# zhu-xlab/tomosar2height

Measured on AMD Instinct MI355X. Metric: training tiles/sec (Berlin crop, cloud-only), higher is better.
Workload: dtype f32; 1 GPU; BASELINE.json configs[1]: Berlin cloud-only, fp32 per-point GEMMs, train_step(tile) per tile, 4 tiles coalesced per forward/backward (Trainer default), N=131072 points/tile, R=256, ALTO depth 5, 512x512 target, optimize_every=64; points_per_tile=131072, optimize_every=64, train_batch=1, coalesce_tiles=4, optimizer=t2h FlatAdamW (one kernel over the flat bucket), parallelism=dp1, rccl_ranks=0, channels_last=True, point_distribution=70 % in 160 buildings + 30 % uniform, grid_convs=conv_bx3.hip: fp32 products from 3 fp16 MFMAs (2-way split, block scales), library_fallbacks=0, hip_graph=False

## Files before the change

### tomosar2height_amd/csrc/conv_bx3.hip

```cpp
#include <stdlib.h>
#include "t2h_common.h"
#include "gemm_args.h"
#include "gemm_tile.h"

namespace t2h {
namespace {

using bf16x8 = __attribute__((ext_vector_type(8))) __bf16;
using f16x8 = __attribute__((ext_vector_type(8))) _Float16;
using f16x2 = __attribute__((ext_vector_type(2))) _Float16;
using bf16x2 = __attribute__((ext_vector_type(2))) __bf16;
using f32x2 = __attribute__((ext_vector_type(2))) float;
using s16x4 = __attribute__((ext_vector_type(4))) short;
using s16x8 = __attribute__((ext_vector_type(8))) short;
typedef __attribute__((address_space(3))) void lds_void;
typedef const __attribute__((address_space(1))) void glb_void;
typedef __attribute__((address_space(3))) s16x4 lds_s16x4;

#ifndef T2H_BX3_BDIRECT
#define T2H_BX3_BDIRECT 1
#endif
constexpr int NT = 256;
constexpr int TW = 32;
constexpr int CC = 32;
// ... 491 lines not shown
        if (t + 1 < T) prefetch(t + 1, pre_m[(t + 1) & 1], pre_o[(t + 1) & 1]);
#pragma unroll
        for (int z = 0; z < 16; ++z)
            patch[((z & 3) + 8 * (z >> 2) + 4 * h) * 36 + r] = H2 ? ldexpf(acc[i][j][z] * winv, -e_cur) : acc[i][j][z];
        float4 bv = make_float4(0.f, 0.f, 0.f, 0.f);
        {
            int col, co;
            tile_off(t, 0, col, co);
            if (p.bias) bv = *reinterpret_cast<const float4 *>(p.bias + co);
        }
#pragma unroll
        for (int pass = 0; pass < 4; ++pass) {
            float4 v = *reinterpret_cast<const float4 *>(patch + (pass * 8 + er) * 36 + ec);
            int col, co;
            const size_t q = tile_off(t, pass, col, co);
            const float4 mk = pre_m[t & 1][pass];
            float4 old = pre_o[t & 1][pass];
            if (rank1 && p.mask) {
                old.x = mk.x > 0.f ? old.x : 0.f; old.y = mk.y > 0.f ? old.y : 0.f;
                old.z = mk.z > 0.f ? old.z : 0.f; old.w = mk.w > 0.f ? old.w : 0.f;
            }
            v.x += bv.x; v.y += bv.y; v.z += bv.z; v.w += bv.w;
            if (UPM == 1) {
                float4 *dst = reinterpret_cast<float4 *>(p.y + q);
                if (accum) { v.x += old.x; v.y += old.y; v.z += old.z; v.w += old.w; }
                if (p.addend) { v.x += mk.x; v.y += mk.y; v.z += mk.z; v.w += mk.w; }
                *dst = v;
                continue;
            }
            if (p.mask) {
                v.x = mk.x > 0.f ? v.x : 0.f; v.y = mk.y > 0.f ? v.y : 0.f;
                v.z = mk.z > 0.f ? v.z : 0.f; v.w = mk.w > 0.f ? v.w : 0.f;
            }
            if (relu) { v.x = relu1(v.x); v.y = relu1(v.y); v.z = relu1(v.z); v.w = relu1(v.w); }
            float4 *dst = reinterpret_cast<float4 *>(ybase + q * p.ldy + col);
            if (accum) { v.x += old.x; v.y += old.y; v.z += old.z; v.w += old.w; }
            *dst = v;
        }
    }
  }
}

struct WgradArgs {
    const float *dy;
    const float *x;
    float *slab;
    float *colslab;
    int H, W, Cin, Cout;
    int n_units, units_per_split;
    int ldx;
    int lddy;
};

template <int COT, int NPL, bool UP = false, int GT = 0>
__global__ __launch_bounds__(NT, 2) void bx3_wgrad_kernel(WgradArgs p) {
    static_assert(!(UP && GT), "UP and GT are different forms");
    constexpr int NTAPS = GT ? GT : (UP ? 4 : 9);
    constexpr int WPC = 4 / COT;
    constexpr int TMAX = (NTAPS + WPC - 1) / WPC;
    constexpr int YS = COT == 1 ? 64 : 64 * COT + 64;
    constexpr int XS = 64;
    constexpr int YPLANE = 32 * YS, XHP = GT ? GT * TW : (UP ? 4 * TW : 3 * (TW + 2)), XPLANE = XHP * XS;
    constexpr int LDS_WORK = NPL * YPLANE + NPL * XPLANE;
    constexpr int LDS_BYTES = LDS_WORK >= 4 * 32 * 36 * 4 ? LDS_WORK : 4 * 32 * 36 * 4;
    constexpr bool H2 = NPL == 2;
    __shared__ __attribute__((aligned(1024))) unsigned char lds[LDS_BYTES + (H2 ? 64 : 0)];
    unsigned char *yimg = lds, *ximg = lds + NPL * YPLANE;
    float *slots = reinterpret_cast<float *>(lds + LDS_BYTES);

    const int tid = threadIdx.x, lane = tid & 63, wave = tid >> 6;
    const int split = GT ? blockIdx.z : blockIdx.x, ci0 = GT ? 0 : blockIdx.y * CC, co0 = (GT ? blockIdx.x : blockIdx.z) * (32 * COT);
    const int u_beg = split * p.units_per_split, u_end = min(p.n_units, u_beg + p.units_per_split);
    const int segs = p.W / TW;

    const int cot = wave / WPC, sub = wave % WPC;
    const int tap_lo = (NTAPS * sub + WPC - 1) / WPC, tap_hi = (NTAPS * (sub + 1) + WPC - 1) / WPC;

    constexpr int XF4 = XHP * 8, XPER = (XF4 + NT - 1) / NT;
    constexpr int YPER = COT;
    float4 xr[XPER], yr[YPER];
    auto load_unit = [&](int u) {
        const int xs = u % segs, row = u / segs;
        const int y = row & (p.H - 1), x0 = xs * TW;
#pragma unroll
        for (int f = 0; f < XPER; ++f) {
            const int idx = tid + f * NT;
            const int px = idx >> 3, c4 = idx & 7;
            const int hy = px / (TW + 2), hx = px - hy * (TW + 2);
            const int gy = y + hy - 1, gx = x0 + hx - 1;
            float4 v = make_float4(0.f, 0.f, 0.f, 0.f);
            if (GT) {
                if (idx < XF4) v = *reinterpret_cast<const float4 *>(p.x + ((size_t)u * TW + (px % TW)) * p.ldx + (px / TW) * 32 + c4 * 4);
            } else if (UP) {
                v = *reinterpret_cast<const float4 *>(p.x + ((size_t)(2 * row + (px >> 6)) * (2 * p.W) + 2 * x0 + (px & 63)) * p.ldx + ci0 + c4 * 4);
            } else if (idx < XF4 && (unsigned)gy < (unsigned)p.H && (unsigned)gx < (unsigned)p.W)
                v = *reinterpret_cast<const float4 *>(p.x + ((size_t)(row + hy - 1) * p.W + gx) * p.ldx + ci0 + c4 * 4);
            xr[f] = v;
        }
#pragma unroll
        for (int f = 0; f < YPER; ++f) {
            const int idx = tid + f * NT;
            const int px = idx / (8 * COT), c4 = idx % (8 * COT);
            yr[f] = *reinterpret_cast<const float4 *>(p.dy + ((size_t)row * p.W + x0 + px) * (GT ? p.lddy : p.Cout) + co0 + c4 * 4);
        }
    };
    float4 csum = make_float4(0.f, 0.f, 0.f, 0.f);
    const bool do_colsum = p.colslab != nullptr && (UP ? blockIdx.z == 0 : blockIdx.y == 0);
    int s_run = E_UNSET, ex_cur = 0, ey_cur = 0;
    auto publish_unit_max = [&](int parity) {
        float mx = 0.f, my = 0.f;
#pragma unroll
        for (int f = 0; f < XPER; ++f) mx = abs4max(mx, xr[f]);
#pragma unroll
        for (int f = 0; f < YPER; ++f) my = abs4max(my, yr[f]);
        mx = wave_max(mx);
        my = wave_max(my);
        if (lane == 0) { slots[(parity * 4 + wave) * 2] = mx; slots[(parity * 4 + wave) * 2 + 1] = my; }
    };
    auto store_unit = [&]() {
#pragma unroll
        for (int f = 0; f < XPER; ++f) {
            const int idx = tid + f * NT;
            if (idx < XF4) {
                const int c4 = idx & 7;
                int px = idx >> 3;
                if (UP) {
                    px = ((px >> 6) * 2 + (px & 1)) * TW + ((px & 63) >> 1);
                    if (do_colsum) { csum.x += xr[f].x; csum.y += xr[f].y; csum.z += xr[f].z; csum.w += xr[f].w; }
                }
                unsigned a1, a2, a3, b1, b2, b3;
                unsigned char *d = ximg + px * XS + c4 * 8;
                if (H2) {
                    split2h(xr[f].x, xr[f].y, ex_cur, a1, a2);
                    split2h(xr[f].z, xr[f].w, ex_cur, b1, b2);
                    *reinterpret_cast<uint2 *>(d) = make_uint2(a1, b1);
                    *reinterpret_cast<uint2 *>(d + XPLANE) = make_uint2(a2, b2);
                    continue;
                }
                split3(xr[f].x, xr[f].y, a1, a2, a3);
                split3(xr[f].z, xr[f].w, b1, b2, b3);
                *reinterpret_cast<uint2 *>(d) = make_uint2(a1, b1);
                if (NPL == 3) {
                    *reinterpret_cast<uint2 *>(d + XPLANE) = make_uint2(a2, b2);
                    *reinterpret_cast<uint2 *>(d + 2 * XPLANE) = make_uint2(a3, b3);
                }
            }
        }
#pragma unroll
        for (int f = 0; f < YPER; ++f) {
            const int idx = tid + f * NT;
            const int px = idx / (8 * COT), c4 = idx % (8 * COT);
            unsigned a1, a2, a3, b1, b2, b3;
            unsigned char *d = yimg + px * YS + c4 * 8;
            if (!UP && do_colsum) { csum.x += yr[f].x; csum.y += yr[f].y; csum.z += yr[f].z; csum.w += yr[f].w; }
            if (H2) {
                split2h(yr[f].x, yr[f].y, ey_cur, a1, a2);
                split2h(yr[f].z, yr[f].w, ey_cur, b1, b2);
                *reinterpret_cast<uint2 *>(d) = make_uint2(a1, b1);
                *reinterpret_cast<uint2 *>(d + YPLANE) = make_uint2(a2, b2);
                continue;
            }
            split3(yr[f].x, yr[f].y, a1, a2, a3);
            split3(yr[f].z, yr[f].w, b1, b2, b3);
            *reinterpret_cast<uint2 *>(d) = make_uint2(a1, b1);
            if (NPL == 3) {
                *reinterpret_cast<uint2 *>(d + YPLANE) = make_uint2(a2, b2);
                *reinterpret_cast<uint2 *>(d + 2 * YPLANE) = make_uint2(a3, b3);
            }
        }
    };

    f32x16 acc[TMAX];
#pragma unroll
    for (int t = 0; t < TMAX; ++t)
#pragma unroll
        for (int z = 0; z < 16; ++z) acc[t][z] = 0.0f;

    const int g = lane >> 4, gi = lane & 15, gq = gi >> 2, gp = gi & 3;
    const int kpix = 8 * (g >> 1) + gq;
    const int choff = (16 * (g & 1) + 4 * gp) * 2;
    auto tr8 = [&](const unsigned char *a, int row_stride) -> bf16x8 {
        const s16x4 lo = __builtin_amdgcn_ds_read_tr16_b64_v4i16((lds_s16x4 *)(a));
        const s16x4 hi = __builtin_amdgcn_ds_read_tr16_b64_v4i16((lds_s16x4 *)(a + 4 * row_stride));
        const s16x8 v = __builtin_shufflevector(lo, hi, 0, 1, 2, 3, 4, 5, 6, 7);
        return *reinterpret_cast<const bf16x8 *>(&v);
    };

    if (u_beg < u_end) load_unit(u_beg);
    if (H2) {
        if (u_beg < u_end) publish_unit_max(u_beg & 1);
        __syncthreads();
    }
    for (int u = u_beg; u < u_end; ++u) {
        if (H2) {
            const float *sl = slots + (u & 1) * 8;
            const int ex_nat = block_exponent(__float_as_uint(fmaxf(fmaxf(sl[0], sl[2]), fmaxf(sl[4], sl[6]))));
            const int ey_nat = block_exponent(__float_as_uint(fmaxf(fmaxf(sl[1], sl[3]), fmaxf(sl[5], sl[7]))));
            if (ex_nat != E_UNSET && ey_nat != E_UNSET && ex_nat + ey_nat < s_run) {
                if (s_run != E_UNSET) {
#pragma unroll
                    for (int t = 0; t < TMAX; ++t)
#pragma unroll
                        for (int z = 0; z < 16; ++z) acc[t][z] = ldexpf(acc[t][z], ex_nat + ey_nat - s_run);
                }
                s_run = ex_nat + ey_nat;
            }
            ex_cur = ex_nat == E_UNSET ? 0 : ex_nat;
            ey_cur = ey_nat == E_UNSET ? 0 : (s_run == E_UNSET ? ey_nat : min(s_run - ex_cur, ey_nat));
        }
        store_unit();
        if (u + 1 < u_end) load_unit(u + 1);
        __syncthreads();
#pragma unroll
        for (int s = 0; s < 2; ++s) {
            bf16x8 af[NPL];
            const unsigned char *ya = yimg + (16 * s + kpix) * YS + cot * 64 + choff;
#pragma unroll
            for (int pl = 0; pl < NPL; ++pl) af[pl] = tr8(ya + pl * YPLANE, YS);
#pragma unroll
            for (int t = 0; t < TMAX; ++t) {
                const int tap = tap_lo + t;
                if (tap < tap_hi) {
                    const int ky = tap / 3, kx = tap - 3 * ky;
                    const unsigned char *xa = ximg + ((UP || GT) ? tap * TW + 16 * s + kpix : ky * (TW + 2) + 16 * s + kpix + kx) * XS + choff;
                    bf16x8 bfr[NPL];
#pragma unroll
                    for (int pl = 0; pl < NPL; ++pl) bfr[pl] = tr8(xa + pl * XPLANE, XS);
                    constexpr int ia[6] = {2, 0, 1, 1, 0, 0}, ib[6] = {0, 2, 1, 0, 1, 0};
                    if (H2) {
#pragma unroll
                        for (int e = 3; e < 6; ++e)
                            acc[t] = __builtin_amdgcn_mfma_f32_32x32x16_f16(*reinterpret_cast<const f16x8 *>(&af[ia[e]]),
                                                                            *reinterpret_cast<const f16x8 *>(&bfr[ib[e]]), acc[t], 0, 0, 0);
                    } else {
#pragma unroll
                        for (int e = (NPL == 3 ? 0 : 5); e < 6; ++e)
                            acc[t] = __builtin_amdgcn_mfma_f32_32x32x16_bf16(af[ia[e]], bfr[ib[e]], acc[t], 0, 0, 0);
                    }
                }
            }
        }
        if (H2 && u + 1 < u_end) publish_unit_max((u + 1) & 1);
        __syncthreads();
    }

    if (do_colsum) {
        float4 *red = reinterpret_cast<float4 *>(lds);
        red[tid] = csum;
        __syncthreads();
        constexpr int CG = UP ? 8 : 8 * COT;
        if (tid < CG) {
            float4 tsum = red[tid];
            for (int j = tid + CG; j < NT; j += CG) { tsum.x += red[j].x; tsum.y += red[j].y; tsum.z += red[j].z; tsum.w += red[j].w; }
            if (UP) *reinterpret_cast<float4 *>(p.colslab + (size_t)split * p.Cin + ci0 + tid * 4) = tsum;
            else *reinterpret_cast<float4 *>(p.colslab + (size_t)split * p.Cout + co0 + tid * 4) = tsum;
        }
        __syncthreads();
    }

    float *patch = reinterpret_cast<float *>(lds) + wave * (32 * 36);
    const int er = lane >> 3, ec = (lane & 7) * 4, r = lane & 31, h = lane >> 5;
    float *sbase = p.slab + (size_t)split * p.Cout * NTAPS * p.Cin;
#pragma unroll
    for (int t = 0; t < TMAX; ++t) {
        const int tap = tap_lo + t;
        if (tap < tap_hi) {
#pragma unroll
            for (int z = 0; z < 16; ++z)
                patch[((z & 3) + 8 * (z >> 2) + 4 * h) * 36 + r] = H2 ? ldexpf(acc[t][z], s_run == E_UNSET ? 0 : -s_run) : acc[t][z];
#pragma unroll
            for (int pass = 0; pass < 4; ++pass) {
                const float4 v = *reinterpret_cast<const float4 *>(patch + (pass * 8 + er) * 36 + ec);
                const int co = co0 + cot * 32 + pass * 8 + er;
                *reinterpret_cast<float4 *>(sbase + ((size_t)co * NTAPS + tap) * p.Cin + ci0 + ec) = v;
            }
        }
    }
}

bool al16(const void *q) { return (uintptr_t)q % 16 == 0; }
bool pow2(int v) { return v > 0 && (v & (v - 1)) == 0; }

int check_bx3(const char *what, int B, int H, int W, int Cin, int Cout) {
    if (B < 1 || !pow2(H) || !pow2(W) || H < 4 || W < TW || H > 32768 || W > 32768 || Cin < 32 || Cout < 32 || Cin % 32 || Cout % 32)
        return fail(T2H_ERR_ARG, "%s: needs power-of-two H >= 4, W >= 32 and Cin, Cout multiples of 32 (B=%d H=%d W=%d %d->%d)", what, B,
                    H, W, Cin, Cout);
    if ((long long)B * H * W > (1LL << 30)) return fail(T2H_ERR_ARG, "%s: more than 2^30 pixels", what);
    return T2H_OK;
}

struct RowsPlan { bool tall; int bn, splits, chunks_per_split; long long tiles; };
RowsPlan bx3_rows_plan(int B, int H, int W, int Kc, int Nc, int ntap = 9, int upm = 0) {
    RowsPlan r{};
    r.bn = Nc % 128 == 0 ? 128 : (Nc % 64 == 0 ? 64 : 32);
    if (upm) {
        r.tall = false;
        const long long row_tiles = (long long)B * (H / 4) * (W / TW);
        if (upm == 1) while (r.bn > 32 && row_tiles * (Nc / r.bn) < 192) r.bn >>= 1;
        r.tiles = row_tiles * (Nc / r.bn);
        r.splits = 1;
        const int nchunk_u = Kc / 64;
        static const long long target_u = 512;
        if (upm == 2 && r.tiles < target_u / 2) {
            long long want = (target_u + r.tiles - 1) / r.tiles;
            if (want > nchunk_u) want = nchunk_u;
            if (want > 32) want = 32;
            r.splits = (int)(want < 1 ? 1 : want);
        }
        r.chunks_per_split = (nchunk_u + r.splits - 1) / r.splits;
        r.splits = (nchunk_u + r.chunks_per_split - 1) / r.chunks_per_split;
        return r;
    }
    static const long long min_tiles8 = env_ll("T2H_BX3_TILES8", 1024);
    const long long tiles8 = H % 8 == 0 ? (long long)B * (H / 8) * (W / TW) * (Nc / r.bn) : 0;
    r.tall = tiles8 >= min_tiles8 && !(ntap == 1 && r.bn == 128);
    r.tiles = r.tall ? tiles8 : (long long)B * (H / 4) * (W / TW) * (Nc / r.bn);
    static const bool narrow = env_flag("T2H_BX3_NARROW", true);
    if (narrow && !r.tall && r.bn == 128 && r.tiles < 256 && Kc <= 128) { r.bn = 64; r.tiles *= 2; }
    r.splits = 1;
    const int nchunk = ntap == 9 ? Kc / (r.tall ? 16 : 32) : Kc / (r.tall ? 32 : 64);
    static const long long target = env_ll("T2H_BX3_ROWS_WGS", 512);
    if (!r.tall && r.tiles < target / 2) {
        long long want = (target + r.tiles - 1) / r.tiles;
        if (want > nchunk) want = nchunk;
        if (want > 32) want = 32;
// ... 50 lines not shown
        e.accum = a.flags & F_ACCUM; e.relu_out = a.flags & F_RELU_OUT;
        a.y = static_cast<float *>(ws); a.bias = nullptr; a.mask = nullptr; a.flags = 0; a.ldy = a.Nc;
    }
    a.splits = r.splits; a.chunks_per_split = r.chunks_per_split; a.ntn_per_wg = 1;
    if (upm == 1) {
        if (r.bn == 128) BX3_LAUNCH_UP(128, 2, 2, 1);
        else if (r.bn == 64) BX3_LAUNCH_UP(64, 4, 1, 1);
        else BX3_LAUNCH_UP(32, 4, 1, 1);
    } else if (upm == 2) {
        if (r.bn == 128) BX3_LAUNCH_UP(128, 2, 2, 2);
        else if (r.bn == 64) BX3_LAUNCH_UP(64, 4, 1, 2);
        else BX3_LAUNCH_UP(32, 4, 1, 2);
    } else if (ntap == 9) {
        if (r.tall) {
            if (r.bn == 128) BX3_LAUNCH(8, 128, 2, 2, 16, 9);
            else if (r.bn == 64) BX3_LAUNCH(8, 64, 4, 1, 16, 9);
            else BX3_LAUNCH(8, 32, 4, 1, 16, 9);
        } else {
            if (r.bn == 128) BX3_LAUNCH(4, 128, 2, 2, 32, 9);
            else if (r.bn == 64) BX3_LAUNCH(4, 64, 4, 1, 32, 9);
            else BX3_LAUNCH(4, 32, 4, 1, 32, 9);
        }
    } else if (ntap == 1 && upm == 0 && npl == 2 && a.Kc == 64 && r.splits == 1 && a.Nc / r.bn >= 8 && persist_n_enabled()) {
        const long long row_tiles = (long long)a.B * (a.H / 4) * (a.W / TW);
        const int pbn = r.bn == 128 ? 64 : r.bn;
        const int ntn = a.Nc / pbn;
        static const long long persist_wgs = env_ll("T2H_BX3_PERSIST_WGS", 2048);
        static const long long min_groups = env_ll("T2H_BX3_PERSIST_MIN_GROUPS", 4);
        long long groups = persist_wgs / (row_tiles > 0 ? row_tiles : 1);
        if (groups < min_groups) groups = min_groups;
        if (groups < 1) groups = 1;
        if (groups > ntn) groups = ntn;
        a.ntn_per_wg = (int)((ntn + groups - 1) / groups);
        groups = (ntn + a.ntn_per_wg - 1) / a.ntn_per_wg;
        const long long pgrid = row_tiles * groups;
        if (pbn == 64) { hipLaunchKernelGGL((bx3_rows_kernel<4, 64, 4, 1, 64, 2, 1, 0, true>), dim3((unsigned)pgrid), dim3(NT), 0, s, a); note_kernel("bx3_rows_kernel<4,64,4,1,64,2,1,0,true>"); }
        else { hipLaunchKernelGGL((bx3_rows_kernel<4, 32, 4, 1, 64, 2, 1, 0, true>), dim3((unsigned)pgrid), dim3(NT), 0, s, a); note_kernel("bx3_rows_kernel<4,32,4,1,64,2,1,0,true>"); }
    } else {
        if (r.tall) {
            if (r.bn == 128) BX3_LAUNCH(8, 128, 2, 2, 32, 1);
            else if (r.bn == 64) BX3_LAUNCH(8, 64, 4, 1, 32, 1);
            else BX3_LAUNCH(8, 32, 4, 1, 32, 1);
        } else {
            if (r.bn == 128) BX3_LAUNCH(4, 128, 2, 2, 64, 1);
            else if (r.bn == 64) BX3_LAUNCH(4, 64, 4, 1, 64, 1);
            else BX3_LAUNCH(4, 32, 4, 1, 64, 1);
        }
    }
    if (int rc = check_launch(what)) return rc;
    if (r.splits > 1) return launch_reduce_rows_epilogue(static_cast<const float *>(ws), r.splits, M * a.Nc, M, a.Nc, e, s);
    return T2H_OK;
}

struct WgradPlan { int cot, splits, units_per_split, n_units; };
WgradPlan bx3_wgrad_plan(int B, int H, int W, int Cin, int Cout) {
    WgradPlan p{};
    p.cot = Cout % 128 == 0 ? 4 : (Cout % 64 == 0 ? 2 : 1);
    p.n_units = B * H * (W / TW);
    const long long groups = (long long)(Cin / CC) * (Cout / (32 * p.cot));
    static const long long forced = env_ll("T2H_BX3_WGRAD_WGS", 0);
    const long long target = forced > 0 ? forced : ((long long)H * W <= 128 * 128 ? 256 : 512);
    long long splits = target / groups;
    if (splits < 1) splits = 1;
    if (splits > p.n_units) splits = p.n_units;
    p.units_per_split = (int)((p.n_units + splits - 1) / splits);
    p.splits = (p.n_units + p.units_per_split - 1) / p.units_per_split;
    return p;
}

}
}

using namespace t2h;

T2H_API int t2h_conv3x3_bx3_supported(int B, int H, int W, int Cin, int Cout) {
    return B >= 1 && pow2(H) && pow2(W) && H >= 4 && W >= TW && H <= 32768 && W <= 32768 && Cin >= 32 && Cout >= 32 && Cin % 32 == 0 &&
           Cout % 32 == 0 && (long long)B * H * W <= (1LL << 30);
}

T2H_API size_t t2h_conv3x3_bx3_weights_bytes(int Cin, int Cout) {
    if (Cin < 32 || Cout < 32 || Cin % 32 || Cout % 32) return 0;
    return (size_t)Cout * 9 * Cin * 6;
}

T2H_API int t2h_conv3x3_bx3_prepare(const float *w, int Cin, int Cout, int transposed, void *wf, t2h_stream_t stream) {
    if (!w || !wf) return fail(T2H_ERR_ARG, "conv3x3_bx3_prepare: null pointer");
    if (Cin < 32 || Cout < 32 || Cin % 32 || Cout % 32 || !al16(wf))
        return fail(T2H_ERR_ARG, "conv3x3_bx3_prepare: Cin=%d, Cout=%d must be multiples of 32, wf 16-byte aligned", Cin, Cout);
    const int Kc = transposed ? Cout : Cin, Nc = transposed ? Cin : Cout;
    const long long total = (long long)(Kc / 16) * 9 * (Nc / 32) * 64;
    const unsigned blocks = (unsigned)((total + 255) / 256);
    if (transposed) hipLaunchKernelGGL(bx3_prepare_kernel<true>, dim3(blocks), dim3(256), 0, as_stream(stream), w, Cin, Cout, static_cast<unsigned *>(wf));
    else hipLaunchKernelGGL(bx3_prepare_kernel<false>, dim3(blocks), dim3(256), 0, as_stream(stream), w, Cin, Cout, static_cast<unsigned *>(wf));
    return check_launch("conv3x3_bx3_prepare");
}

T2H_API size_t t2h_conv3x3_bx3_fwd_workspace_bytes(int B, int H, int W, int Cin, int Cout) {
    if (!t2h_conv3x3_bx3_supported(B, H, W, Cin, Cout)) return 0;
    const RowsPlan r = bx3_rows_plan(B, H, W, Cin, Cout);
    return r.splits > 1 ? (size_t)r.splits * B * H * W * Cout * sizeof(float) : 0;
}

T2H_API size_t t2h_conv3x3_bx3_dgrad_workspace_bytes(int B, int H, int W, int Cin, int Cout) {
    if (!t2h_conv3x3_bx3_supported(B, H, W, Cin, Cout)) return 0;
    const RowsPlan r = bx3_rows_plan(B, H, W, Cout, Cin);
    return r.splits > 1 ? (size_t)r.splits * B * H * W * Cin * sizeof(float) : 0;
}

T2H_API int t2h_conv3x3_bx3_fwd(const float *x, const void *wf, const float *bias, float *y, int B, int H, int W, int Cin, int Cout,
                                int flags, void *workspace, size_t workspace_bytes, t2h_stream_t stream) {
    if (!x || !wf || !y) return fail(T2H_ERR_ARG, "conv3x3_bx3_fwd: null pointer");
    if (int rc = check_bx3("conv3x3_bx3_fwd", B, H, W, Cin, Cout)) return rc;
// ... 11 lines not shown
    if (!dy || !wf_t || !dx) return fail(T2H_ERR_ARG, "conv3x3_bx3_dgrad: null pointer");
    if (int rc = check_bx3("conv3x3_bx3_dgrad", B, H, W, Cin, Cout)) return rc;
    if (!al16(dy) || !al16(wf_t) || !al16(dx) || (mask && !al16(mask))) return fail(T2H_ERR_ARG, "conv3x3_bx3_dgrad: pointers must be 16-byte aligned");
    RowsArgs a{};
    a.x = dy; a.wf = static_cast<const unsigned *>(wf_t); a.bias = nullptr; a.mask = mask; a.y = dx;
    a.B = B; a.H = H; a.W = W; a.Kc = Cout; a.Nc = Cin; a.ldx = Cout; a.ldy = Cin; a.ldm = Cin;
    a.flags = (flags & T2H_ACCUM) ? F_ACCUM : 0;
    a.wscale = f16_trailer(wf_t, (size_t)Cout * 9 * Cin * 4);
    return launch_rows(a, npl_of(flags), workspace, workspace_bytes, as_stream(stream), "conv3x3_bx3_dgrad");
}

T2H_API int t2h_conv3x3_bx3_dgrad_rank1_supported(int B, int H, int W, int Cin, int Cout) {
    if (!t2h_conv3x3_bx3_supported(B, H, W, Cin, Cout)) return 0;
    return bx3_rows_plan(B, H, W, Cout, Cin).splits == 1;
}

T2H_API int t2h_conv3x3_bx3_dgrad_rank1(const float *dy, const void *wf_t, float *dx, const float *mask, const float *g, const float *w1,
                                        int B, int H, int W, int Cin, int Cout, int flags, t2h_stream_t stream) {
    if (!dy || !wf_t || !dx || !g || !w1) return fail(T2H_ERR_ARG, "conv3x3_bx3_dgrad_rank1: null pointer");
    if (int rc = check_bx3("conv3x3_bx3_dgrad_rank1", B, H, W, Cin, Cout)) return rc;
    if (!t2h_conv3x3_bx3_dgrad_rank1_supported(B, H, W, Cin, Cout))
        return fail(T2H_ERR_ARG, "conv3x3_bx3_dgrad_rank1: this shape splits its reduction (use t2h_conv3x3_bx3_dgrad with T2H_ACCUM)");
    if (flags & T2H_ACCUM) return fail(T2H_ERR_ARG, "conv3x3_bx3_dgrad_rank1: the rank-1 term takes the place of the accumulated values");
    if (!al16(dy) || !al16(wf_t) || !al16(dx) || (mask && !al16(mask)) || !al16(w1))
        return fail(T2H_ERR_ARG, "conv3x3_bx3_dgrad_rank1: pointers must be 16-byte aligned");
    RowsArgs a{};
    a.x = dy; a.wf = static_cast<const unsigned *>(wf_t); a.bias = nullptr; a.mask = mask; a.y = dx;
    a.B = B; a.H = H; a.W = W; a.Kc = Cout; a.Nc = Cin; a.ldx = Cout; a.ldy = Cin; a.ldm = Cin;
    a.flags = 0; a.r1_g = g; a.r1_w = w1;
    a.wscale = f16_trailer(wf_t, (size_t)Cout * 9 * Cin * 4);
    return launch_rows(a, npl_of(flags), nullptr, 0, as_stream(stream), "conv3x3_bx3_dgrad_rank1");
}

T2H_API size_t t2h_conv3x3_bx3_wgrad_workspace_bytes(int B, int H, int W, int Cin, int Cout) {
    if (!t2h_conv3x3_bx3_supported(B, H, W, Cin, Cout)) return 0;
    WgradPlan p = bx3_wgrad_plan(B, H, W, Cin, Cout);
    return (size_t)p.splits * ((size_t)Cout * 9 * Cin + Cout) * sizeof(float);
}

T2H_API int t2h_conv3x3_bx3_wgrad(const float *dy, const float *x, float *dw, float *db, int B, int H, int W, int Cin, int Cout,
                                  int flags, void *workspace, size_t workspace_bytes, t2h_stream_t stream) {
    if (!dy || !x || !dw) return fail(T2H_ERR_ARG, "conv3x3_bx3_wgrad: null pointer");
    if (int rc = check_bx3("conv3x3_bx3_wgrad", B, H, W, Cin, Cout)) return rc;
    if (!al16(dy) || !al16(x)) return fail(T2H_ERR_ARG, "conv3x3_bx3_wgrad: pointers must be 16-byte aligned");
    const size_t need = t2h_conv3x3_bx3_wgrad_workspace_bytes(B, H, W, Cin, Cout);
    if (!workspace || workspace_bytes < need || !al16(workspace))
        return fail(T2H_ERR_WORKSPACE, "conv3x3_bx3_wgrad: workspace %zu < %zu bytes", workspace_bytes, need);
    hipStream_t s = as_stream(stream);
    WgradPlan p = bx3_wgrad_plan(B, H, W, Cin, Cout);
    const int Ncols = 9 * Cin;
    float *slab = static_cast<float *>(workspace);
    float *colslab = slab + (size_t)p.splits * Cout * Ncols;
    WgradArgs a{};
    a.dy = dy; a.x = x; a.slab = slab; a.colslab = db ? colslab : nullptr;
    a.H = H; a.W = W; a.Cin = Cin; a.Cout = Cout; a.n_units = p.n_units; a.units_per_split = p.units_per_split; a.ldx = Cin;
    dim3 grid(p.splits, Cin / CC, Cout / (32 * p.cot));
    if (grid.y > 65535 || grid.z > 65535) return fail(T2H_ERR_ARG, "conv3x3_bx3_wgrad: too many channel chunks");
    if (flags & T2H_F16X2) {
        if (p.cot == 4) { hipLaunchKernelGGL((bx3_wgrad_kernel<4, 2>), grid, dim3(NT), 0, s, a); note_kernel("bx3_wgrad_kernel<4,2,false,0>"); }
        else if (p.cot == 2) { hipLaunchKernelGGL((bx3_wgrad_kernel<2, 2>), grid, dim3(NT), 0, s, a); note_kernel("bx3_wgrad_kernel<2,2,false,0>"); }
        else { hipLaunchKernelGGL((bx3_wgrad_kernel<1, 2>), grid, dim3(NT), 0, s, a); note_kernel("bx3_wgrad_kernel<1,2,false,0>"); }
    } else if (flags & T2H_BF16) {
        if (p.cot == 4) { hipLaunchKernelGGL((bx3_wgrad_kernel<4, 1>), grid, dim3(NT), 0, s, a); note_kernel("bx3_wgrad_kernel<4,1,false,0>"); }
        else if (p.cot == 2) { hipLaunchKernelGGL((bx3_wgrad_kernel<2, 1>), grid, dim3(NT), 0, s, a); note_kernel("bx3_wgrad_kernel<2,1,false,0>"); }
        else { hipLaunchKernelGGL((bx3_wgrad_kernel<1, 1>), grid, dim3(NT), 0, s, a); note_kernel("bx3_wgrad_kernel<1,1,false,0>"); }
    } else {
        if (p.cot == 4) { hipLaunchKernelGGL((bx3_wgrad_kernel<4, 3>), grid, dim3(NT), 0, s, a); note_kernel("bx3_wgrad_kernel<4,3,false,0>"); }
        else if (p.cot == 2) { hipLaunchKernelGGL((bx3_wgrad_kernel<2, 3>), grid, dim3(NT), 0, s, a); note_kernel("bx3_wgrad_kernel<2,3,false,0>"); }
        else { hipLaunchKernelGGL((bx3_wgrad_kernel<1, 3>), grid, dim3(NT), 0, s, a); note_kernel("bx3_wgrad_kernel<1,3,false,0>"); }
    }
    if (int rc = check_launch("conv3x3_bx3_wgrad")) return rc;
    return launch_reduce_slabs(slab, p.splits, (long long)Cout * Ncols, Cout, Ncols, Ncols, (flags & T2H_ACCUM) ? 1 : 0, dw, colslab, db, s,
                               0, 0, (flags & T2H_DEFER_REDUCE) != 0);
}

T2H_API int t2h_gemm_bx3_supported(int64_t M, int K, int N) {
    return M >= 128 && M % 128 == 0 && M <= (1LL << 30) && K >= 64 && K % 64 == 0 && N >= 32 && N % 32 == 0;
}

T2H_API size_t t2h_gemm_bx3_weights_bytes(int K, int N) {
    if (K < 16 || N < 32 || K % 16 || N % 32) return 0;
    return (size_t)K * N * 6;
}

T2H_API int t2h_gemm_bx3_prepare(const float *w, int ldw, int K, int N, int w_is_kn, void *wf, t2h_stream_t stream) {
    if (!w || !wf) return fail(T2H_ERR_ARG, "gemm_bx3_prepare: null pointer");
    if (K < 16 || N < 32 || K % 16 || N % 32 || !al16(wf) || ldw < (w_is_kn ? N : K))
        return fail(T2H_ERR_ARG, "gemm_bx3_prepare: K=%d must be a multiple of 16, N=%d of 32, ldw=%d at least the row length", K, N, ldw);
    const long long total = (long long)(K / 16) * (N / 32) * 64;
    const unsigned blocks = (unsigned)((total + 255) / 256);
    if (w_is_kn) hipLaunchKernelGGL(bx3_prepare_gemm_kernel<true>, dim3(blocks), dim3(256), 0, as_stream(stream), w, K, N, ldw, static_cast<unsigned *>(wf));
    else hipLaunchKernelGGL(bx3_prepare_gemm_kernel<false>, dim3(blocks), dim3(256), 0, as_stream(stream), w, K, N, ldw, static_cast<unsigned *>(wf));
    return check_launch("gemm_bx3_prepare");
}

T2H_API size_t t2h_gemm_bx3_workspace_bytes(int64_t M, int K, int N) {
    if (!t2h_gemm_bx3_supported(M, K, N)) return 0;
    const RowsPlan r = bx3_rows_plan(1, (int)(M / 32), 32, K, N, 1);
    return r.splits > 1 ? (size_t)r.splits * M * N * sizeof(float) : 0;
}

T2H_API int t2h_gemm_bx3(const float *x, int ldx, const void *wf, const float *bias, const float *mask, int ldm, float *y, int ldy,
                         int64_t M, int K, int N, int flags, void *workspace, size_t workspace_bytes, t2h_stream_t stream,
                         const int32_t *n_rows) {
    if (!x || !wf || !y) return fail(T2H_ERR_ARG, "gemm_bx3: null pointer");
    if (!t2h_gemm_bx3_supported(M, K, N))
        return fail(T2H_ERR_ARG, "gemm_bx3: needs M %% 128 == 0, K %% 64 == 0, N %% 32 == 0 (M=%lld K=%d N=%d)", (long long)M, K, N);
    if (ldx < K || ldy < N || ldx % 4 || ldy % 4 || (mask && (ldm < N || ldm % 4)) || !al16(x) || !al16(wf) || !al16(y) || (bias && !al16(bias)) ||
        (mask && !al16(mask)))
        return fail(T2H_ERR_ARG, "gemm_bx3: rows must be 16-byte aligned and at least K / N floats long");
    RowsArgs a{};
    a.x = x; a.wf = static_cast<const unsigned *>(wf); a.bias = bias; a.mask = mask; a.y = y;
    a.B = 1; a.H = (int)(M / 32); a.W = 32; a.Kc = K; a.Nc = N; a.ldx = ldx; a.ldy = ldy; a.ldm = ldm;
    a.flags = ((flags & T2H_RELU_OUT) ? F_RELU_OUT : 0) | ((flags & T2H_ACCUM) ? F_ACCUM : 0);
    a.wscale = f16_trailer(wf, (size_t)K * N * 4);
    a.row_limit = n_rows;
    return launch_rows(a, npl_of(flags), workspace, workspace_bytes, as_stream(stream), "gemm_bx3", 1);
}

static int gemm_wgrad_splits(int64_t M, int N) {
    static const long long target = env_ll("T2H_GEMM_BX3_WGRAD_WGS", 4096);
    const long long groups = N / 64, units = M / TW;
    long long splits = (target + groups - 1) / groups;
// ... 221 lines not shown
```

### tomosar2height_amd/switches.py

```python
import os

SWITCHES = {
    "T2H_LIBRARY": dict(kind="str", default=None, owner="_lib.py", scope="env",
        doc="path of another build of the same ABI (A/B runs of a kernel change; a site-specific install path)"),
    "T2H_ALLOW_LIBRARY_FALLBACK": dict(kind="flag", default=False, owner="_lib.py", scope="env",
        doc="1: shapes without a t2h kernel run on MIOpen / rocBLAS / ATen (counted) instead of raising"),
    "T2H_BUILD_JOBS": dict(kind="int", default=6, owner="csrc/build.py", scope="env", doc="sources compiled in parallel"),
    "T2H_LLVM_BIN": dict(kind="str", default="/opt/rocm/lib/llvm/bin", owner="csrc/build.py", scope="env",
        doc="clang / lld / clang-offload-bundler of compile_through_assembly"),
    "T2H_CACHE_READY": dict(kind="flag", default=True, owner="_lib.py", scope="lab",
        doc="0: lazily filled cache entries are NOT waited for across streams -- the r04-r06 race, kept to show its tests catching it"),
    "T2H_POISON_LDS": dict(kind="flag", default=False, owner="_lib.py", scope="lab",
        doc="1: NaN patterns into every free CU's LDS before every entry point (t2h_debug_poison_lds)"),
    "T2H_SEAM_SYNC_CHECK": dict(kind="flag", default=False, owner="ops.py", scope="lab",
        doc="1 (debugging): every seam call waits for its own index check and raises at the call, like torch_scatter"),
    "T2H_DIRECT_ACCUM": dict(kind="flag", default=True, owner="trainer.py",
        doc="0: autograd's own gradient accumulation instead of kernels adding straight into the bucket"),
    "T2H_OVERLAP_WGRAD": dict(kind="flag", default=True, owner="trainer.py",
        doc="0: the weight-gradient GEMMs stay on the step's stream (1: a side stream, joined after the backward)"),
    "T2H_OVERLAP_CONV_WGRAD": dict(kind="flag", default=True, owner="trainer.py",
        doc="0: the convolutions' weight gradients stay on the step's stream (1: beside the next data gradients)"),
    "T2H_PIPELINE_TILES": dict(kind="flag", default=True, owner="trainer.py",
        doc="0: one tile after the other (1: tile i + 1's forward beside tile i's backward, two streams)"),
    "T2H_PIPELINE_MICRO_BATCHES": dict(kind="flag", default=True, owner="trainer.py", doc="0: a micro-batch of a window runs on the caller's stream alone"),
    "T2H_COALESCE_TILES": dict(kind="int", default=4, owner="trainer.py", covered_by="tests/test_launch_census.py",
        doc="single tiles issued as one ragged micro-batch of this many; 1: the strict B = 1 step"),
    "T2H_COMPOSE_CACHE": dict(kind="flag", default=True, owner="trainer.py",
        doc="0: the composed maps of the deferred levels are back-propagated per tile, not once per step"),
    "T2H_BATCH_REDUCE": dict(kind="flag", default=True, owner="trainer.py",
        doc="0: one slab reduction launch per layer instead of one batched launch per pass (only without the side streams)"),
    "T2H_HIP_CONV": dict(kind="flag", default=True, owner="grid.py",
        doc="0: every convolution stays on MIOpen (an explicit request, so it also allows the fallbacks)"),
    "T2H_CONV_PRECISION": dict(kind=("fp32", "bf16x3", "f16x2", "bf16"), default="f16x2", owner="grid.py",
        doc="arithmetic of the 3x3 / transposed convolutions and the wide grid-side products (grid.py, above CONV_PRECISION)"),
    "T2H_BX3_MIN_PIXELS": dict(kind="int", default=1024, owner="grid.py", doc="smaller planes stay on conv.hip"),
    "T2H_BX3_WGRAD": dict(kind="flag", default=True, owner="grid.py", doc="0: weight gradients stay on conv.hip"),
    "T2H_UPCONV_BX3": dict(kind="flag", default=True, owner="grid.py", doc="0: transposed convolutions stay on conv.hip (fp32 MFMA)"),
    "T2H_HEAD_RANK1": dict(kind="flag", default=True, owner="grid.py",
        doc="0: the 1 x 1 head writes its share of the decoder gradients, the data gradients accumulate onto it (bit-identical)"),
    "T2H_OVERLAP_CONV_MAX_PIXELS": dict(kind="int", default=512 * 512, owner="grid.py",
        doc="planes up to here send their weight gradients to the trainer's side stream"),
    "T2H_CONV_ROWS_WGS_SMALL": dict(kind="int", default=768, owner="csrc/conv.hip", library=True,
        doc="workgroups the split reduction aims at, up to 16384 output rows"),
    "T2H_CONV_ROWS_WGS_LARGE": dict(kind="int", default=512, owner="csrc/conv.hip", library=True,
        doc="workgroups the split reduction aims at, above 16384 output rows"),
    "T2H_UPCONV_FWD_TILES": dict(kind="int", default=256, owner="csrc/conv.hip", library=True,
        doc="the transposed convolution's column tiles narrow until there are this many tiles"),
    "T2H_CONV_WGRAD_WGS": dict(kind="int", default=0, owner="csrc/conv.hip", library=True,
        doc="workgroups the weight gradient aims at (0: 512 for planes up to 128 x 128, else 1024)"),
    "T2H_BX3_TILES8": dict(kind="int", default=1024, owner="csrc/conv_bx3.hip", library=True, doc="8-row tiles from this many tiles on"),
    "T2H_BX3_NARROW": dict(kind="flag", default=True, owner="csrc/conv_bx3.hip", library=True,
        doc="0: small planes with short reductions keep 128-column tiles and split the reduction"),
    "T2H_BX3_ROWS_WGS": dict(kind="int", default=512, owner="csrc/conv_bx3.hip", library=True, doc="workgroups the split reduction aims at"),
    "T2H_BX3_WGRAD_WGS": dict(kind="int", default=0, owner="csrc/conv_bx3.hip", library=True,
        doc="workgroups the split weight gradient aims at (0: 256 for planes up to 128 x 128, else 512)"),
    "T2H_BX3_UPWGRAD_WGS": dict(kind="int", default=0, owner="csrc/conv_bx3.hip", library=True,
        doc="workgroups the transposed convolution's weight gradient aims at (0: 256)"),
    "T2H_GEMM_BX3": dict(kind="flag", default=True, owner="mlp.py", doc="0: the grid-side products of the deferred point update stay on the fp32 MFMA kernels"),
    "T2H_GEMM_BX3_MIN_N": dict(kind="int", default=64, owner="mlp.py", doc="fewer output columns stay on the fp32 kernels"),
    "T2H_GEMM_BX3_MIN_K": dict(kind="int", default=128, owner="mlp.py", doc="shorter reductions stay on the fp32 kernels"),
    "T2H_GEMM_BX3_WGRAD": dict(kind="flag", default=False, owner="mlp.py",
        doc="1: the wide weight gradients dW = dY^T X on the split kernels too (t2h_gemm_bx3_wgrad)"),
    "T2H_GEMM_BX3_WGRAD_MIN_N": dict(kind="int", default=1024, owner="mlp.py", doc="... from this many columns of dY on"),
    "T2H_GEMM_BX3_WGRAD_MIN_M": dict(kind="int", default=4096, owner="mlp.py", doc="... and from this many rows on"),
    "T2H_GEMM_BX3_WGRAD_WGS": dict(kind="int", default=4096, owner="csrc/conv_bx3.hip", library=True,
        doc="workgroups that weight gradient's row split aims at"),
    "T2H_BX3_PERSIST_N": dict(kind="flag", default=True, owner="csrc/conv_bx3.hip", library=True, mirror="mlp.py",
        doc="0: no persistent form (rows staged and split once per workgroup, reused for all its column tiles) for one-chunk "
            "reductions into a wide matrix; mlp.py routes such shapes by it"),
    "T2H_BX3_PERSIST_WGS": dict(kind="int", default=2048, owner="csrc/conv_bx3.hip", library=True,
        doc="workgroups of the persistent form: column groups = this / row tiles"),
    "T2H_BX3_PERSIST_MIN_GROUPS": dict(kind="int", default=4, owner="csrc/conv_bx3.hip", library=True,
        doc="... but at least this many column groups however many row tiles there are"),
    "T2H_GEMM_DMA": dict(kind="flag", default=True, owner="csrc/gemm.hip", library=True,
        doc="0: the register-staged kernels instead of the LDS-DMA ones (forward, data and TN weight gradient)"),
    "T2H_SKINNY": dict(kind="flag", default=True, owner="csrc/gemm.hip", library=True,
        doc="0: no 64 x 64 x 32 tiles for 33 .. 64 output columns from a long reduction"),
    "T2H_SMALLM_BK": dict(kind="int", default=64, owner="csrc/gemm.hip", library=True, doc="slab depth of the small-tile kernels for few rows (64 / 32 / 16)"),
    "T2H_KWAVES_MIN_K": dict(kind="int", default=256, owner="csrc/gemm.hip", library=True,
        doc="the four waves of a workgroup split reductions from this depth on"),
    "T2H_KWAVES_MAX_TILES": dict(kind="int", default=1024, owner="csrc/gemm.hip", library=True, doc="... for outputs of up to this many 32 x 32 tiles"),
    "T2H_KWAVES_WGRAD_MAX_ROWS": dict(kind="int", default=1024, owner="csrc/gemm.hip", library=True,
        doc="the weight gradient takes that one-launch form up to this many rows"),
    "T2H_FUSED_TRUNK": dict(kind="flag", default=True, owner="mlp.py", doc="0: one GEMM launch per Linear + pool kernels"),
    "T2H_TRUNK_FUSED": dict(kind=("auto", "1", "0"), default="auto", owner="mlp.py",
        doc="auto and 1: the whole trunk forward in one launch from _TRUNK_FUSED_MIN_ROWS rows on; 0: one launch per block"),
    "T2H_TRUNK_FUSED_STRIDE": dict(kind="int", default=0, owner="mlp.py",
        doc="rows per fixed-stride window of the one launch without unit bounds (0: 96; at most 128)"),
    "T2H_TRUNK_UNIT_BOUNDS": dict(kind="flag", default=True, owner="mlp.py",
        doc="0: fixed-stride windows looked up in the kernel (1: greedy units built once per tile index)"),
    "T2H_GRID_FIRST_MIN_RATIO": dict(kind="float", default=4.0, owner="mlp.py", doc="points per pixel from which fc_comm.0 runs on the pixels; 0: never"),
    "T2H_DEFER_MIN_CHANNELS": dict(kind="int", default=128, owner="deferred.py", doc="deferral starts at the first level with this many channels; 0: off"),
    "T2H_FUSED_SAMPLE_BWD": dict(kind="flag", default=True, owner="deferred.py", doc="0: separate gather + sample adjoint"),
    "T2H_SIGN_BITS": dict(kind="flag", default=True, owner="deferred.py", doc="0: keep the hidden activations for the mask"),
    "T2H_ON_CHIP_HIDDEN": dict(kind="flag", default=True, owner="deferred.py", doc="0: sample kernel + per-cell sum kernel"),
    "T2H_ON_CHIP_MIN_PTS": dict(kind="float", default=8.0, owner="deferred.py",
        doc="points per cell from which the on-chip walk is taken (it is sequential inside a cell)"),
    "T2H_COMPACT_SUMS": dict(kind="flag", default=True, owner="deferred.py",
        doc="0: one row per CELL in the sum matrices of every resolution (1: the finest deferred resolution holds one row per OCCUPIED cell)"),
    "T2H_SAMPLE_ADJOINT": dict(kind="flag", default=True, owner="ops.py", doc="0: no sample backward through the cached transposed matrix"),
    "T2H_SAMPLE_ADJOINT_MAX_ROWS": dict(kind="float", default=4.0, owner="ops.py",
        doc="rows per pixel above which t2h_sample_bwd's gather / per-cell partials stay"),
    "T2H_CELLS_MFMA": dict(kind="flag", default=True, owner="csrc/point_grid.hip", library=True, mirror="deferred.py",
        doc="0: the VALU form of the sample adjoint's per-cell partials; deferred.py's bit mask needs the matrix-core form"),
    "T2H_CELLS_MIN_WGS": dict(kind="int", default=4096, owner="csrc/point_grid.hip", library=True, doc="workgroups the per-cell partials' row splits aim at"),
    "T2H_CELLS_TABLE": dict(kind="int", default=1, owner="csrc/point_grid.hip", library=True,
        doc="0: no cell table in the matrix-core partials (the r04 walk)"),
    "T2H_FPS_SLICE": dict(kind="int", default=None, owner="pointops.py", covered_by="tests/test_pnpp_gpu.py",
# ... 16 lines not shown
```

Measured before the change: 195.9 tiles/s.

## Swap operand roles in 3x3 weight-gradient kernel when Cin permits wider tiles

When Cin is divisible by a larger power of two than Cout, the 3x3 weight-gradient kernel now treats the input activations as the wide (output-channel) side and dY as the halo side. The result is written back transposed with the tap flipped, and the bias column sum is taken from the interior of the haloed tile. Wider workgroup tiles along the larger channel dimension are meant to raise data reuse per MFMA and cut redundant halo staging. This adds a new template variant and a transposed store path, with an env switch to disable it.

```diff
diff --git a/tomosar2height_amd/csrc/conv_bx3.hip b/tomosar2height_amd/csrc/conv_bx3.hip
--- a/tomosar2height_amd/csrc/conv_bx3.hip
+++ b/tomosar2height_amd/csrc/conv_bx3.hip
@@ -567,9 +567,10 @@
     int lddy;
 };
 
-template <int COT, int NPL, bool UP = false, int GT = 0>
+template <int COT, int NPL, bool UP = false, int GT = 0, bool SW = false>
 __global__ __launch_bounds__(NT, 2) void bx3_wgrad_kernel(WgradArgs p) {
     static_assert(!(UP && GT), "UP and GT are different forms");
+    static_assert(!(SW && (UP || GT)), "SW is the 3 x 3 form with its operands swapped");
     constexpr int NTAPS = GT ? GT : (UP ? 4 : 9);
     constexpr int WPC = 4 / COT;
     constexpr int TMAX = (NTAPS + WPC - 1) / WPC;
@@ -620,7 +621,10 @@
         }
     };
     float4 csum = make_float4(0.f, 0.f, 0.f, 0.f);
-    const bool do_colsum = p.colslab != nullptr && (UP ? blockIdx.z == 0 : blockIdx.y == 0);
+    const bool do_colsum = p.colslab != nullptr && ((UP || SW) ? blockIdx.z == 0 : blockIdx.y == 0);
+    constexpr int sw_first = 8 * (TW + 3) - NT;
+    static_assert(!SW || (sw_first >= 0 && sw_first < NT && XPER >= 3), "SW: one interior float4 per thread");
+    const unsigned sw_m1 = (unsigned)((sw_first - 1 - tid) >> 31);
     int s_run = E_UNSET, ex_cur = 0, ey_cur = 0;
     auto publish_unit_max = [&](int parity) {
         float mx = 0.f, my = 0.f;
@@ -642,6 +646,11 @@
                 if (UP) {
                     px = ((px >> 6) * 2 + (px & 1)) * TW + ((px & 63) >> 1);
                     if (do_colsum) { csum.x += xr[f].x; csum.y += xr[f].y; csum.z += xr[f].z; csum.w += xr[f].w; }
+                }
+                if (SW && f == 1 && do_colsum) {
+                    auto pick = [&](float a, float b) { return __uint_as_float((__float_as_uint(a) & sw_m1) | (__float_as_uint(b) & ~sw_m1)); };
+                    csum.x += pick(xr[1].x, xr[2].x); csum.y += pick(xr[1].y, xr[2].y);
+                    csum.z += pick(xr[1].z, xr[2].z); csum.w += pick(xr[1].w, xr[2].w);
                 }
                 unsigned a1, a2, a3, b1, b2, b3;
                 unsigned char *d = ximg + px * XS + c4 * 8;
@@ -667,7 +676,7 @@
             const int px = idx / (8 * COT), c4 = idx % (8 * COT);
             unsigned a1, a2, a3, b1, b2, b3;
             unsigned char *d = yimg + px * YS + c4 * 8;
-            if (!UP && do_colsum) { csum.x += yr[f].x; csum.y += yr[f].y; csum.z += yr[f].z; csum.w += yr[f].w; }
+            if (!UP && !SW && do_colsum) { csum.x += yr[f].x; csum.y += yr[f].y; csum.z += yr[f].z; csum.w += yr[f].w; }
             if (H2) {
                 split2h(yr[f].x, yr[f].y, ey_cur, a1, a2);
                 split2h(yr[f].z, yr[f].w, ey_cur, b1, b2);
@@ -763,11 +772,11 @@
         float4 *red = reinterpret_cast<float4 *>(lds);
         red[tid] = csum;
         __syncthreads();
-        constexpr int CG = UP ? 8 : 8 * COT;
+        constexpr int CG = (UP || SW) ? 8 : 8 * COT;
         if (tid < CG) {
             float4 tsum = red[tid];
             for (int j = tid + CG; j < NT; j += CG) { tsum.x += red[j].x; tsum.y += red[j].y; tsum.z += red[j].z; tsum.w += red[j].w; }
-            if (UP) *reinterpret_cast<float4 *>(p.colslab + (size_t)split * p.Cin + ci0 + tid * 4) = tsum;
+            if (UP || SW) *reinterpret_cast<float4 *>(p.colslab + (size_t)split * p.Cin + ci0 + tid * 4) = tsum;
             else *reinterpret_cast<float4 *>(p.colslab + (size_t)split * p.Cout + co0 + tid * 4) = tsum;
         }
         __syncthreads();
@@ -781,11 +790,19 @@
         const int tap = tap_lo + t;
         if (tap < tap_hi) {
 #pragma unroll
-            for (int z = 0; z < 16; ++z)
-                patch[((z & 3) + 8 * (z >> 2) + 4 * h) * 36 + r] = H2 ? ldexpf(acc[t][z], s_run == E_UNSET ? 0 : -s_run) : acc[t][z];
+            for (int z = 0; z < 16; ++z) {
+                const float v = H2 ? ldexpf(acc[t][z], s_run == E_UNSET ? 0 : -s_run) : acc[t][z];
+                if (SW) patch[r * 36 + (z & 3) + 8 * (z >> 2) + 4 * h] = v;
+                else patch[((z & 3) + 8 * (z >> 2) + 4 * h) * 36 + r] = v;
+            }
 #pragma unroll
             for (int pass = 0; pass < 4; ++pass) {
                 const float4 v = *reinterpret_cast<const float4 *>(patch + (pass * 8 + er) * 36 + ec);
+                if (SW) {
+                    const int lco = ci0 + pass * 8 + er;
+                    *reinterpret_cast<float4 *>(sbase + ((size_t)lco * NTAPS + (NTAPS - 1 - tap)) * p.Cout + co0 + cot * 32 + ec) = v;
+                    continue;
+                }
                 const int co = co0 + cot * 32 + pass * 8 + er;
                 *reinterpret_cast<float4 *>(sbase + ((size_t)co * NTAPS + tap) * p.Cin + ci0 + ec) = v;
             }
@@ -942,12 +959,17 @@
     return T2H_OK;
 }
 
-struct WgradPlan { int cot, splits, units_per_split, n_units; };
+struct WgradPlan { int cot, splits, units_per_split, n_units, cot_name; bool swap; };
+int wgrad_cot(int c) { return c % 128 == 0 ? 4 : (c % 64 == 0 ? 2 : 1); }
 WgradPlan bx3_wgrad_plan(int B, int H, int W, int Cin, int Cout) {
     WgradPlan p{};
-    p.cot = Cout % 128 == 0 ? 4 : (Cout % 64 == 0 ? 2 : 1);
+    static const bool may_swap = env_flag("T2H_BX3_WGRAD_SWAP", true);
+    p.cot_name = wgrad_cot(Cout);
+    p.swap = may_swap && wgrad_cot(Cin) > p.cot_name;
+    p.cot = p.swap ? wgrad_cot(Cin) : p.cot_name;
     p.n_units = B * H * (W / TW);
-    const long long groups = (long long)(Cin / CC) * (Cout / (32 * p.cot));
+    const int wide = p.swap ? Cin : Cout, halo = p.swap ? Cout : Cin;
+    const long long groups = (long long)(halo / CC) * (wide / (32 * p.cot));
     static const long long forced = env_ll("T2H_BX3_WGRAD_WGS", 0);
     const long long target = forced > 0 ? forced : ((long long)H * W <= 128 * 128 ? 256 : 512);
     long long splits = target / groups;
@@ -1065,23 +1087,27 @@
     float *slab = static_cast<float *>(workspace);
     float *colslab = slab + (size_t)p.splits * Cout * Ncols;
     WgradArgs a{};
-    a.dy = dy; a.x = x; a.slab = slab; a.colslab = db ? colslab : nullptr;
-    a.H = H; a.W = W; a.Cin = Cin; a.Cout = Cout; a.n_units = p.n_units; a.units_per_split = p.units_per_split; a.ldx = Cin;
-    dim3 grid(p.splits, Cin / CC, Cout / (32 * p.cot));
+    a.slab = slab; a.colslab = db ? colslab : nullptr;
+    a.H = H; a.W = W; a.n_units = p.n_units; a.units_per_split = p.units_per_split;
+    if (p.swap) { a.dy = x; a.x = dy; a.Cout = Cin; a.Cin = Cout; a.ldx = Cout; }
+    else { a.dy = dy; a.x = x; a.Cout = Cout; a.Cin = Cin; a.ldx = Cin; }
+    dim3 grid(p.splits, a.Cin / CC, a.Cout / (32 * p.cot));
     if (grid.y > 65535 || grid.z > 65535) return fail(T2H_ERR_ARG, "conv3x3_bx3_wgrad: too many channel chunks");
-    if (flags & T2H_F16X2) {
-        if (p.cot == 4) { hipLaunchKernelGGL((bx3_wgrad_kernel<4, 2>), grid, dim3(NT), 0, s, a); note_kernel("bx3_wgrad_kernel<4,2,false,0>"); }
-        else if (p.cot == 2) { hipLaunchKernelGGL((bx3_wgrad_kernel<2, 2>), grid, dim3(NT), 0, s, a); note_kernel("bx3_wgrad_kernel<2,2,false,0>"); }
-        else { hipLaunchKernelGGL((bx3_wgrad_kernel<1, 2>), grid, dim3(NT), 0, s, a); note_kernel("bx3_wgrad_kernel<1,2,false,0>"); }
-    } else if (flags & T2H_BF16) {
-        if (p.cot == 4) { hipLaunchKernelGGL((bx3_wgrad_kernel<4, 1>), grid, dim3(NT), 0, s, a); note_kernel("bx3_wgrad_kernel<4,1,false,0>"); }
-        else if (p.cot == 2) { hipLaunchKernelGGL((bx3_wgrad_kernel<2, 1>), grid, dim3(NT), 0, s, a); note_kernel("bx3_wgrad_kernel<2,1,false,0>"); }
-        else { hipLaunchKernelGGL((bx3_wgrad_kernel<1, 1>), grid, dim3(NT), 0, s, a); note_kernel("bx3_wgrad_kernel<1,1,false,0>"); }
-    } else {
-        if (p.cot == 4) { hipLaunchKernelGGL((bx3_wgrad_kernel<4, 3>), grid, dim3(NT), 0, s, a); note_kernel("bx3_wgrad_kernel<4,3,false,0>"); }
-        else if (p.cot == 2) { hipLaunchKernelGGL((bx3_wgrad_kernel<2, 3>), grid, dim3(NT), 0, s, a); note_kernel("bx3_wgrad_kernel<2,3,false,0>"); }
-        else { hipLaunchKernelGGL((bx3_wgrad_kernel<1, 3>), grid, dim3(NT), 0, s, a); note_kernel("bx3_wgrad_kernel<1,3,false,0>"); }
-    }
+#define BX3_WGRAD_LAUNCH(COT_, NPL_, SW_) hipLaunchKernelGGL((bx3_wgrad_kernel<COT_, NPL_, false, 0, SW_>), grid, dim3(NT), 0, s, a)
+#define BX3_WGRAD_LAUNCH_COT(NPL_)                                                                                           \
+    do {                                                                                                                    \
+        if (p.swap) { if (p.cot == 4) BX3_WGRAD_LAUNCH(4, NPL_, true); else BX3_WGRAD_LAUNCH(2, NPL_, true); }              \
+        else if (p.cot == 4) BX3_WGRAD_LAUNCH(4, NPL_, false);                                                              \
+        else if (p.cot == 2) BX3_WGRAD_LAUNCH(2, NPL_, false);                                                              \
+        else BX3_WGRAD_LAUNCH(1, NPL_, false);                                                                              \
+        note_kernel(p.cot_name == 4 ? "bx3_wgrad_kernel<4," #NPL_ ",false,0>"                                               \
+                                    : (p.cot_name == 2 ? "bx3_wgrad_kernel<2," #NPL_ ",false,0>" : "bx3_wgrad_kernel<1," #NPL_ ",false,0>")); \
+    } while (0)
+    if (flags & T2H_F16X2) BX3_WGRAD_LAUNCH_COT(2);
+    else if (flags & T2H_BF16) BX3_WGRAD_LAUNCH_COT(1);
+    else BX3_WGRAD_LAUNCH_COT(3);
+#undef BX3_WGRAD_LAUNCH_COT
+#undef BX3_WGRAD_LAUNCH
     if (int rc = check_launch("conv3x3_bx3_wgrad")) return rc;
     return launch_reduce_slabs(slab, p.splits, (long long)Cout * Ncols, Cout, Ncols, Ncols, (flags & T2H_ACCUM) ? 1 : 0, dw, colslab, db, s,
                                0, 0, (flags & T2H_DEFER_REDUCE) != 0);
diff --git a/tomosar2height_amd/switches.py b/tomosar2height_amd/switches.py
--- a/tomosar2height_amd/switches.py
+++ b/tomosar2height_amd/switches.py
@@ -54,6 +54,9 @@
     "T2H_BX3_ROWS_WGS": dict(kind="int", default=512, owner="csrc/conv_bx3.hip", library=True, doc="workgroups the split reduction aims at"),
     "T2H_BX3_WGRAD_WGS": dict(kind="int", default=0, owner="csrc/conv_bx3.hip", library=True,
         doc="workgroups the split weight gradient aims at (0: 256 for planes up to 128 x 128, else 512)"),
+    "T2H_BX3_WGRAD_SWAP": dict(kind="flag", default=True, owner="csrc/conv_bx3.hip", library=True,
+        covered_by="tests/test_conv_bx3_wgrad_swap_gpu.py",
+        doc="0: no 3x3 weight gradient runs with its operands' roles swapped (1: X on the wide side where Cin allows wider workgroups than Cout)"),
     "T2H_BX3_UPWGRAD_WGS": dict(kind="int", default=0, owner="csrc/conv_bx3.hip", library=True,
         doc="workgroups the transposed convolution's weight gradient aims at (0: 256)"),
     "T2H_GEMM_BX3": dict(kind="flag", default=True, owner="mlp.py", doc="0: the grid-side products of the deferred point update stay on the fp32 MFMA kernels"),
```

Result: no change. 197.1 tiles/s (median of 6 runs) (+0.6%).
